# vedantsawal/Cost-and-Carbon-Aware-Kubernetes-Autoscaler

Hardware: AMD Instinct MI355X
Metric: policy-evaluated cluster-steps/sec (higher is better)
Workload: dtype int32+int64+f64; 1 GPU; config2: 1e5 clusters x 1 deployment x 1440 one-minute steps, HPA + peak/off-peak, 16-type catalog; scenarios_per_gpu=100000, steps_per_rollout=1440, mode=trajectory, schedule=lane-skewed (single deployment), trace_layout=wave-tiled [wave][T][lanes] (built by the first rollout), parallelism=scenario-sharded x1

## Files before the change

### cost-and-carbon-aware-kubernetes-autoscaler_amd/csrc/abi_debug.cpp

```cpp
#include <algorithm>
#include <cstdio>
#include <vector>

#include "ctx.h"
#include "host_rules.h"

using namespace ccka;

int stamps_buffer(ccka_ctx* c, unsigned long long** out) {
  if (!c->d_stamps.reserve(12)) return fail(c, CCKA_ENOMEM, "stamps alloc");
  HIPCHK(c, hipMemsetAsync(c->d_stamps, 0, 12 * sizeof(unsigned long long), c->stream));
  *out = c->d_stamps;
  return CCKA_OK;
}

extern "C" {

int ccka_debug_copy_gbs(ccka_ctx* c, int64_t bytes, int32_t reps, double* gbs) {
  if (!c || !gbs || bytes < (1 << 20) || reps < 1 || reps > 64) return CCKA_EINVAL;
  (void)hipSetDevice(c->device);
  bytes &= ~(int64_t)4095;
  DevBuf<char> a, b;
  if (!a.resize(bytes) || !b.resize(bytes))
    return fail(c, CCKA_ENOMEM, "copy probe alloc (2 x %lld bytes)", (long long)bytes);
// ... 28 lines not shown

int ccka_debug_engine(ccka_ctx* c, int32_t mode) {
  if (!c || mode < 0 || mode > 3) return CCKA_EINVAL;
  c->sk_coop_f2 = mode == 3;
  c->engine_mode = mode == 3 ? 0 : mode;
  return CCKA_OK;
}

int ccka_debug_last_engine(ccka_ctx* c, int32_t* engine, double* table_ms) {
  if (!c) return CCKA_EINVAL;
  if (engine) *engine = c->last_engine;
  if (table_ms) *table_ms = c->last_table_ms;
  return CCKA_OK;
}

int ccka_debug_last_plan(ccka_ctx* c, int32_t out[12]) {
  static_assert(PLAN_FIELDS == 12, "ccka_debug_last_plan's out[12]");
  if (!c || !out) return CCKA_EINVAL;
  if (!c->ran || c->last_engine == 3 || c->last_engine == 4) return fail(c, CCKA_ESTATE, "no whole-horizon rollout ran last");
  std::copy(c->last_plan, c->last_plan + PLAN_FIELDS, out);
  return CCKA_OK;
}

int ccka_debug_pg_chunk(ccka_ctx* c, int64_t rows) {
  if (!c || rows < 0) return CCKA_EINVAL;
  c->pg_chunk = rows;
  return CCKA_OK;
}

int ccka_debug_policy_table(ccka_ctx* c, int32_t on) {
  if (!c) return CCKA_EINVAL;
  c->pol_table_off = on == 0;
  return CCKA_OK;
}

int ccka_debug_policy_fused(ccka_ctx* c, int32_t on) {
  if (!c) return CCKA_EINVAL;
  c->pol_fused_off = on == 0;
  return CCKA_OK;
}

int ccka_debug_policy_graph(ccka_ctx* c, int32_t on) {
  if (!c) return CCKA_EINVAL;
  c->pol_graph_off = on == 0;
  return CCKA_OK;
}

int ccka_debug_lpw(ccka_ctx* c, int32_t lpw) {
  if (!c || lpw < 0 || lpw > 64) return CCKA_EINVAL;
  c->lpw = lpw;
  return CCKA_OK;
}

int ccka_debug_trace_flat(ccka_ctx* c, int32_t on) {
  if (!c) return CCKA_EINVAL;
  c->trace_flat = on != 0;
  return CCKA_OK;
}

int ccka_debug_occ(ccka_ctx* c, int32_t occ) {
  if (!c || occ < 0 || occ > 3 || occ == 1) return CCKA_EINVAL;
  c->occ = occ;
  return CCKA_OK;
}

int ccka_debug_mlp_tile(ccka_ctx* c, int32_t tile) {
  if (!c || (tile != 16 && tile != 32)) return CCKA_EINVAL;
  c->mlp_tile = tile;
  return CCKA_OK;
}

int ccka_debug_mlp_stamps(ccka_ctx* c, int32_t enable) {
  if (!c) return CCKA_EINVAL;
  c->mlp_stamps = enable != 0;
  return CCKA_OK;
}

int ccka_debug_stamps(ccka_ctx* c, unsigned long long* out8) {
  if (!c || !out8 || !c->d_stamps) return CCKA_EINVAL;
  HIPCHK(c, hipMemcpy(out8, c->d_stamps, 12 * sizeof(unsigned long long), hipMemcpyDeviceToHost));
  return CCKA_OK;
}

int ccka_debug_totals(ccka_ctx* c, const int64_t* cost, const int32_t* slo, const int64_t* pend_min,
                      const int32_t* nmin_spot, const int32_t* nmin_od, const int32_t* launches,
                      const int32_t* deletions, const double* energy, const double* gco2, int64_t n,
                      ccka_totals* out) {
  if (!c || !cost || !slo || !pend_min || !nmin_spot || !nmin_od || !launches || !deletions || !energy || !gco2 ||
      !out || n < 1 || n > (int64_t)1 << 31)
    return CCKA_EINVAL;
  (void)hipSetDevice(c->device);
  DevBuf<char> d_res;
  if (!d_res.resize(carve_results(nullptr, n, nullptr))) return fail(c, CCKA_ENOMEM, "totals columns (%lld)", (long long)n);
  ResultPtrs r{};
  carve_results(d_res, n, &r);
  struct { void* dst; const void* src; size_t sz; } m[] = {
      {r.cost, cost, 8}, {r.slo, slo, 4}, {r.pend_min, pend_min, 8}, {r.nmin_spot, nmin_spot, 4},
      {r.nmin_od, nmin_od, 4}, {r.launches, launches, 4}, {r.deletions, deletions, 4}, {r.energy, energy, 8},
      {r.gco2, gco2, 8}};
  for (auto& x : m) HIPCHK(c, hipMemcpyAsync(x.dst, x.src, (size_t)n * x.sz, hipMemcpyHostToDevice, c->stream));
  const int rc = totals_of(c, r, n, out);
  (void)hipStreamSynchronize(c->stream);
  return rc;
}

int ccka_debug_traj_stage(ccka_ctx* c, int64_t records) {
// ... 33 lines not shown
```

### cost-and-carbon-aware-kubernetes-autoscaler_amd/csrc/abi_rollout.cpp

```cpp
#include <algorithm>
#include <cstddef>
#include <cstring>

#include "ctx.h"
#include "host_rules.h"

using namespace ccka;

static int32_t d1_lpw(const ccka_ctx* c) {
  if (c->lpw > 0) return c->lpw;
  const int64_t slots = 2LL * 4 * c->cus;
  return (int32_t)std::min<int64_t>(64, std::max<int64_t>(32, (c->N + slots - 1) / slots));
}

static int d1_trace_tile(ccka_ctx* c) {
  if (!c->d1_world || c->hw.n_deploy != 1 || c->n_traces > 0 || !c->have_load) return CCKA_OK;
  const int32_t lpw = d1_lpw(c);
  if (c->load_w_lpw == lpw && c->d_load_w) return CCKA_OK;
  const int64_t cnt = trace_tile_count(c->N, c->hw.n_steps, lpw);
  c->load_w_lpw = 0;
  if (!c->d_load_w.resize(cnt)) return CCKA_OK;
  HIPCHK(c, launch_trace_tile(c->d_load, c->d_load_w, c->N, c->hw.n_steps, lpw, c->stream));
  HIPCHK(c, hipStreamSynchronize(c->stream));
  c->load_w_lpw = lpw;
// ... 132 lines not shown
  if (dmax > 4) return false;
  if (k.nsub != 1 || k.hlen != 0 || !k.all_hours || (k.ablate & ~16) != 0) return false;
  if (w.disrupt_ext & (CCKA_DISRUPT_DRIFT | CCKA_DISRUPT_REPLACE | CCKA_DISRUPT_MULTI)) return false;
  for (int d = 0; d < w.n_deploy; ++d) {
    const int sc = w.deploy[d].scaler;
    if (sc != CCKA_SCALER_HPA && sc != CCKA_SCALER_STATIC) return false;
    if (sc != CCKA_SCALER_HPA) continue;
    const ccka_deployment& dp = w.deploy[d];
    if (dp.target_util_pct <= 0 || dp.target_util_pct > kSkMax16) return false;
    if (!(dp.tolerance >= 0.0 && dp.tolerance < 1.0)) return false;
    if (dp.max_replicas > kSkMax16 || dp.replicas0 > kSkMax16) return false;
  }
  if (c->sc_target_max > kSkMax16 || c->sc_maxr_max > kSkMax16) return false;
  return true;
}

extern "C" {

int ccka_rollout_async(ccka_ctx* c, int32_t trajectory) {
  if (!c) return CCKA_EINVAL;
  if (!c->have_world || !c->have_sc) return fail(c, CCKA_ESTATE, "world/scenarios not set");
  if (!c->have_load) return fail(c, CCKA_ESTATE, "no load traces (ccka_set_load / ccka_gen_load)");
  (void)hipSetDevice(c->device);
  const ccka_world& w = c->hw;
  int block = 256;
  size_t lds = 0;
  int rc;
  KParams k;
  if ((rc = setup_general(c, trajectory, k, &block, &lds)) != CCKA_OK) return rc;
  int32_t* const plan = c->last_plan;
  std::fill(plan, plan + PLAN_FIELDS, -1);
  plan[PLAN_TRACE_MOD] = k.trace_mod != 0;
  if (c->engine_mode == 0 && c->d1_world && !c->d1_ready && (rc = d1_prepare(c)) != CCKA_OK) return rc;
  if (c->engine_mode == 0 && c->d1_world && c->d1_ok && !c->detail_on) {
    const TableParams tp = table_params(c, c->d_wc1000, c->NW, c->d_table, c->d_jtab);
    D1Params p = c->d1;
    p.load = c->d_load; p.price = c->d_price; p.ci_gpwmin = c->d_ci_gpwmin; p.acc = c->d_acc;
    p.table = c->d_table; p.jtab = c->d_jtab;
    p.region = c->d_region; p.target = c->d_target; p.maxr = c->d_maxr; p.down_stab = c->d_dstab;
    p.reset_ca = c->d_resetca; p.pswitch = c->d_pswitch; p.wci = c->d_wci; p.cap_sel = c->d_capsel;
    p.res = k.res; p.traj = k.traj;
    p.N = c->N;
    p.NL = k.NL;
    p.trace_mod = k.trace_mod;
    p.first_id = k.first_id;
    p.NW = c->NW;
    p.occ = c->occ > 0 ? c->occ : 2;
    p.lpw = d1_lpw(c);
    if (!c->trace_flat) {
      if ((rc = d1_trace_tile(c)) != CCKA_OK) return rc;
      if (c->load_w_lpw == p.lpw && c->d_load_w && p.trace_mod == 0) p.load_w = c->d_load_w;
    }
    p.ablate = k.ablate;
    if ((k.ablate & 16) && (rc = stamps_buffer(c, &p.stamps)) != CCKA_OK) return rc;
    HIPCHK(c, hipEventRecord(c->ev0, c->stream));
    HIPCHK(c, launch_table(tp, c->stream));
    if (p.replace || p.multi) {
      TableParams t2 = tp;
      t2.wc1000 = c->d_wc0;
      t2.NW = 1;
      t2.offer = 1;
      t2.table = c->d_table2;
      t2.jtab = c->d_jtab2;
      HIPCHK(c, launch_table(t2, c->stream));
      p.table2 = c->d_table2;
    }
    HIPCHK(c, hipEventRecord(c->ev_mid, c->stream));
    HIPCHK(c, launch_rollout_d1(p, c->stream, plan));
    plan[PLAN_D1_NW] = c->NW;
    plan[PLAN_D1_NZI] = p.NZI;
    plan[PLAN_D1_JT] = p.JT;
    HIPCHK(c, hipEventRecord(c->ev1, c->stream));
    c->last_engine = 2;
    c->traj_nt = true;
  } else {
    if ((k.ablate & 16) && (rc = stamps_buffer(c, &k.stamps)) != CCKA_OK) return rc;
    const bool sk = sk_eligible(c, k);
    if (sk) {
      if ((rc = sk_trace(c)) != CCKA_OK) return rc;
      if (c->load_nt_dp) k.load_nt = c->d_load_nt;
      int dmax, nmax;
      kernel_dims(w.n_deploy, w.max_nodes, &dmax, &nmax);
      const size_t col = ((lds + 15) & ~(size_t)15), need = (size_t)nmax * (7 + dmax) * block * 4;
      if (!c->sk_coop_f2 && rollout_sk_lane_f2() && w.n_types <= 64 && col + need <= 160 * 1024) {
        k.lds_lclaims = (int32_t)col;
        lds = col + need;
      }
    }
    HIPCHK(c, hipEventRecord(c->ev0, c->stream));
    HIPCHK(c, hipEventRecord(c->ev_mid, c->stream));
    if (sk) HIPCHK(c, launch_rollout_sk(k, block, lds, c->stream));
    else HIPCHK(c, launch_rollout(k, block, lds, c->stream));
    HIPCHK(c, hipEventRecord(c->ev1, c->stream));
    plan[PLAN_GRID] = (int32_t)((c->N + block - 1) / block);
    plan[PLAN_SPAN] = k.span;
    plan[PLAN_ALL_HOURS] = k.all_hours;
    plan[PLAN_HLEN] = k.hlen;
    plan[PLAN_LDS] = (int32_t)lds;
    plan[PLAN_LCLAIMS] = k.lds_lclaims >= 0;
    c->last_engine = sk ? 5 : 1;
    c->traj_nt = sk;
  }
  c->traj_valid = trajectory != 0;
  c->detail_valid = c->detail_on;
  c->ran = true;
  return CCKA_OK;
}

int ccka_set_detail(ccka_ctx* c, int32_t on) {
  if (!c) return CCKA_EINVAL;
  c->detail_on = on != 0;
  return CCKA_OK;
}

int ccka_get_detail(ccka_ctx* c, ccka_detail* out, int64_t count) {
  if (!c || !out) return CCKA_EINVAL;
  if (!c->ran || !c->detail_valid) return fail(c, CCKA_ESTATE, "last rollout recorded no detail (ccka_set_detail)");
  if (count != c->N) return fail(c, CCKA_EINVAL, "detail count %lld != %lld scenarios", (long long)count, (long long)c->N);
  (void)hipSetDevice(c->device);
  HIPCHK(c, hipMemcpy2DAsync(out, sizeof(ccka_detail), c->d_detail, sizeof(DetailDev), sizeof(ccka_detail), (size_t)count,
                             hipMemcpyDeviceToHost, c->stream));
  HIPCHK(c, hipStreamSynchronize(c->stream));
  return CCKA_OK;
}
// ... 199 lines not shown
```

### cost-and-carbon-aware-kubernetes-autoscaler_amd/csrc/ctx.h

```cpp
#pragma once
#include <hip/hip_runtime.h>
#include <rccl/rccl.h>

#include <cstdint>
#include <string>
#include <vector>

#include "../../include/ccka.h"
#include "devbuf.h"
#include "kparams.h"

#pragma GCC visibility push(hidden)

struct ccka_ctx {
  template <class T>
  using Buf = ccka::DevBuf<T>;

  int device = 0;
  hipStream_t stream = nullptr;
  hipEvent_t ev0 = nullptr, ev_mid = nullptr, ev1 = nullptr;
  std::string err;
  int cus = 0;
  char name[128] = {0};
  bool have_world = false;
// ... 17 lines not shown
  Buf<uint8_t> d_capsel;
  Buf<int32_t> d_load;
  bool have_load = false;
  Buf<int32_t> d_load_w;
  int32_t load_w_lpw = 0;
  Buf<int32_t> d_load_nt;
  int32_t load_nt_dp = 0;
  bool trace_flat = false;
  Buf<char> d_res;
  ccka::ResultPtrs res{};
  Buf<ccka_traj_rec> d_traj;
  bool traj_valid = false;
  bool traj_nt = false;
  Buf<ccka_traj_rec> d_traj_t;
  int64_t traj_stage = 0;
  Buf<long long> d_parts;
  Buf<ccka_totals> d_totals;
  Buf<int32_t> d_sinq;
  ncclComm_t comm = nullptr;
  double last_ms = 0.0;
  double last_table_ms = 0.0;
  bool ran = false;
  bool d1_world = false;
  bool d1_ready = false;
  bool d1_ok = false;
  bool sc_maxr_ok = true;
  int sc_dstab_max = -1;
  int sc_target_max = -1;
  int sc_maxr_max = -1;
  Buf<int2> d_hist;
  uint32_t sc_capsel_or = 0;
  int sc_pswitch_any = -1;
  ccka::D1Params d1{};
  std::vector<uint32_t> zmasks;
  std::vector<double> h_cw;
  Buf<long long> d_acc;
  Buf<int32_t> d_order;
  Buf<int32_t> d_cap1s;
  Buf<int32_t> d_cap1t;
  Buf<uint32_t> d_zmasks;
  Buf<double> d_wc1000;
  Buf<uint8_t> d_wci;
  Buf<int2> d_table;
  Buf<int32_t> d_jtab;
  Buf<int2> d_table2;
  Buf<int32_t> d_jtab2;
  Buf<double> d_wc0;
  int JT = 0, NW = 0;
  int engine_mode = 0;
  bool sk_coop_f2 = false;
  int32_t ablate = 0;
  Buf<unsigned long long> d_stamps;
  int lpw = 0;
  int occ = 0;
  int mlp_stamps = 0;
  Buf<ccka_grid_stats> d_gstats;
  Buf<ccka_grid_stats> d_gcand;
  Buf<ccka_grid_stats> d_ggather;
  Buf<int64_t> d_gcounts;
  Buf<int32_t> d_gn;
  Buf<uint8_t> d_gflags;
  Buf<ccka_grid_stats> d_gfront;
  Buf<ccka_timeline_row> d_tlrows;
  Buf<int64_t> d_snap;
  bool have_snap = false;
  int64_t snap_first = 0, snap_n = 0, snap_grid_size = 0, snap_traces = 0;
  Buf<ccka_paired_row> d_prows;
  Buf<uint32_t> d_pflag;
  bool mlp_have_w = false;
  Buf<ccka::mlp_bf16x8> d_w1f;
  Buf<ccka::mlp_bf16x8> d_w2f;
  Buf<ccka::mlp_bf16x8> d_w3f;
  Buf<ccka::mlp_bf16x8> d_w1g;
  Buf<ccka::mlp_bf16x8> d_w2g;
  Buf<ccka::mlp_bf16x8> d_w3g;
  int mlp_tile = 16;
  Buf<float> d_mb;
  Buf<uint16_t> d_mx;
  Buf<float> d_my;
  int64_t mlp_n = 0;
  int last_engine = 0;
  int32_t last_plan[ccka::PLAN_FIELDS] = {0};
  Buf<int32_t> d_pol_state;
  Buf<int16_t> d_pol_target;
  Buf<double> d_pol_cw;
  Buf<int16_t> d_rec_target;
  Buf<double> d_rec_cw;
  bool pol_rec_valid = false;
  bool pol_feat_on = false;
  hipGraphExec_t pol_graph = nullptr;
  std::vector<unsigned char> pol_graph_key;
  bool pol_graph_off = false;
  bool pol_fused_off = false;
  bool pol_table_off = false;
  int64_t pg_chunk = 0;
  int64_t pg_mpad = 0;
  Buf<int2> d_ptable;
  Buf<int32_t> d_pjtab;
  Buf<double> d_pwc;
  Buf<uint16_t> d_feat_rec;
  Buf<ccka::mlp_bf16x8> d_w2b;
  Buf<ccka::mlp_bf16x8> d_w3b;
  Buf<uint8_t> d_pg_act;
  Buf<float> d_pg_coef;
  Buf<uint64_t> d_pg_seed;
  uint64_t pg_seed_host = 0;
// ... 45 lines not shown
```

### cost-and-carbon-aware-kubernetes-autoscaler_amd/csrc/host_rules.h

```cpp
#pragma once
#include <cstdint>

#include "../../include/ccka.h"

namespace ccka {

inline const char* trace_gen_invalid(const ccka_trace_gen& g) {
  typedef __int128 i128;
  const int64_t wb = (int64_t)g.base_hi - g.base_lo, wa = (int64_t)g.amp_hi_pm - g.amp_lo_pm;
  if (wb < 0 || wa < 0) return "a range has hi < lo";
  if (wb + 1 > INT32_MAX || wa + 1 > INT32_MAX) return "a range's width + 1 exceeds int32";
  if (g.burst_len < 0) return "burst_len < 0";
  if (g.burst_len > INT32_MAX - 1439) return "bstart + burst_len can exceed int32";
  auto mag = [](int32_t lo, int32_t hi) {
    const i128 a = lo < 0 ? -(i128)lo : (i128)lo, b = hi < 0 ? -(i128)hi : (i128)hi;
    return a > b ? a : b;
  };
  const i128 lim = INT64_MAX;
  const i128 B = mag(g.base_lo, g.base_hi), A = mag(g.amp_lo_pm, g.amp_hi_pm);
  const i128 P1 = B * (65536000 + 65536 * A);
  if (P1 > lim) return "base * (65536000 + amp * SIN) can leave int64";
  const i128 V1 = P1 / 65536000;
  const i128 P2 = V1 * (37837000 + 131072 * mag(g.noise_pm, g.noise_pm));
  if (P2 > lim) return "v * (37837000 + noise * e) can leave int64";
  const i128 V2 = P2 / 37837000;
  if (V2 * mag(g.burst_mult_pm, g.burst_mult_pm) > lim) return "v * burst_mult can leave int64";
  return nullptr;
}

constexpr int32_t kMaxStartMinute = INT32_MAX - 65535;
constexpr int32_t kMaxProvisionDelay = 0x7ffffffe - 65534;

inline const char* world_timing_invalid(const ccka_world& w) {
  if (w.n_steps < 1 || w.n_steps > 65535) return "n_steps out of range";
  if (w.start_minute < 0 || w.provision_delay_steps < 0) return "negative timing";
  if (w.start_minute > kMaxStartMinute) return "start_minute + n_steps can leave int32";
  if (w.provision_delay_steps > kMaxProvisionDelay) return "a ready step t + provision_delay_steps can reach 0x7fffffff";
  if (w.peak_start_min < 0 || w.peak_start_min > 1440) return "peak_start_min outside [0, 1440]";
  if (w.peak_end_min < 0 || w.peak_end_min > 1440) return "peak_end_min outside [0, 1440]";
  return nullptr;
}

constexpr int64_t kTrajStageRecs = int64_t(4) << 20;

inline int64_t traj_stage_cap(int64_t N, int64_t count, int64_t stage) {
  const int64_t lim = stage > 0 ? stage : kTrajStageRecs;
  const int64_t cap = count < lim ? count : lim;
  return cap > N ? cap : N;
}

inline int64_t trace_tile_count(int64_t N, int64_t T, int64_t lpw) { return T * ((N + lpw - 1) / lpw * lpw); }
inline int64_t trace_nt_count(int64_t NL, int64_t T, int64_t DP) { return NL * T * DP; }

}
```

### cost-and-carbon-aware-kubernetes-autoscaler_amd/csrc/kparams.h

```cpp
#pragma once
#include <hip/hip_runtime.h>
#include <stddef.h>
#include <stdint.h>

#include "../../include/ccka.h"

namespace ccka {

struct DetailDev {
  ccka_detail d;
  int64_t e_hour[CCKA_MAX_POOLS];
  int64_t base_e_hour;
};

__host__ __device__ constexpr int64_t state_words(int dmax, int nmax) {
  return (int64_t)dmax * (5 + 2 * CCKA_HIST) + 5 * CCKA_MAX_POOLS + (int64_t)nmax * (6 + dmax) + 36;
}

__host__ __device__ constexpr int hist_entries(int window_s, int sync_s) {
  return window_s > sync_s ? (window_s - 1) / sync_s : 0;
}

struct ResultPtrs {
  int64_t* cost;
// ... 139 lines not shown
struct D1Patch {
  int32_t policy, cas, zi, cm;
};

struct D1Params {
  const int32_t* load;
  const int32_t* load_w;
  const int32_t* price;
  const double* ci_gpwmin;
  const long long* acc;
  const int2* table;
  const int32_t* jtab;
  const uint8_t* region;
  const int16_t* target;
  const int16_t* maxr;
  const int16_t* down_stab;
  const int16_t* reset_ca;
  const uint8_t* pswitch;
  const uint8_t* wci;
  const uint8_t* cap_sel;
  ResultPtrs res;
  ccka_traj_rec* traj;
  int64_t N;
  int64_t NL, trace_mod, first_id;
  int32_t lpw;
  int32_t occ;
  int32_t bdef;
  int32_t T, K, Z, R, NP, maxn, NZI, NW, JT;
  int32_t start_minute, peak_start, peak_end, pswitch0, delay;
  int32_t base_nodes, base_type, slo_util, pdb_pct, pdb_member;
  int32_t replicas0, minr, maxr0, target0, req_cpu, limit, dstab0, reset_ca0, capsel0;
  double tol_lo, tol_hi;
  long long base_nw;
  int32_t ablate;
  unsigned long long* stamps;
  D1Rule up, dn;
  int32_t budget[CCKA_MAX_POOLS];
  D1Patch patch[CCKA_MAX_POOLS][4];
  int32_t drift;
  uint32_t zml[16];
  int32_t drift_on;
  int32_t replace;
  const int2* table2;
  int32_t lds_tab;
  int32_t nsub;
  int32_t he4;
  int32_t multi;
  int32_t keda;
  int32_t k_thr;
  int32_t k_act;
  int32_t k_cds;
  int32_t k_min;
  int32_t k_max;
};
static_assert(sizeof(D1Params) == 1048 && offsetof(D1Params, traj) == 232, "D1Params: the kernels' argument layout");

struct TableParams {
  const int32_t* price;
  const double* ci_gpwh;
  const ccka_itype* types;
  const int32_t* order;
  const int32_t* cap1s;
  const int32_t* cap1t;
  const uint32_t* zmasks;
  const double* wc1000;
  int2* table;
  int32_t* jtab;
  int32_t K, Z, R, NZI, NW, JT;
  int32_t offer;
};

hipError_t launch_table(const TableParams& t, hipStream_t s);
hipError_t launch_trace_tile(const int32_t* in, int32_t* out, int64_t N, int64_t T, int32_t lpw, hipStream_t s);

struct GridSrc {
  const int64_t* cost;
  const double* gco2;
  const int32_t* slo;
  const double* energy;
  int64_t grid_size, first_grid, n_grids;
};
hipError_t launch_grid_stats(const GridSrc& g, ccka_grid_stats* out, hipStream_t s);
struct GridSel {
  GridSrc g;
  int64_t rank[4];
  int32_t kind[4];
};
hipError_t launch_grid_select(const GridSel& q, ccka_grid_stats* out, hipStream_t s);
hipError_t launch_copy16(const void* in, void* out, int64_t bytes, int cus, hipStream_t s);
hipError_t launch_pareto(const ccka_grid_stats* in, int n, const int32_t* n_dev, uint8_t* flags,
                         ccka_grid_stats* out, int32_t* count_dev, hipStream_t s);
hipError_t launch_pareto_union(const ccka_grid_stats* gathered, const int64_t* counts, int ranks, int cap,
                               ccka_grid_stats* out, int32_t* n_dev, hipStream_t s);

struct MlpParams {
  const uint16_t* x;
  float* y;
  const mlp_bf16x8* w1f;
  const mlp_bf16x8* w2f;
  const mlp_bf16x8* w3f;
  const float *b1, *b2, *b3;
  int64_t N;
  unsigned long long* stamps;
  const mlp_bf16x8* w1g;
  const mlp_bf16x8* w2g;
  const mlp_bf16x8* w3g;
};
hipError_t launch_mlp(const MlpParams& p, int cus, hipStream_t s);
// ... 91 lines not shown
```

### cost-and-carbon-aware-kubernetes-autoscaler_amd/csrc/rollout_d1.hip

```cpp
#include <hip/hip_runtime.h>
#include <stdint.h>

#include "../../include/ccka.h"
#include "d1_common.h"
#include "kparams.h"

#pragma clang fp contract(off)

namespace ccka {

namespace {

struct Best {
  double s;
  int k;
  int info;
  int price;
};

__device__ __forceinline__ bool better(double s2, int k2, double s, int k) {
  return s2 < s || (s2 == s && k2 < k);
}

__device__ __forceinline__ void take_if_better(Best& a, const Best& b) {
  if (better(b.s, b.k, a.s, a.k)) a = b;
}

__device__ __forceinline__ Best shfl_up_best(const Best& a, int off) {
  Best o;
  o.s = __shfl_up(a.s, off);
  o.k = __shfl_up(a.k, off);
  o.info = __shfl_up(a.info, off);
  o.price = __shfl_up(a.price, off);
  return o;
}

__device__ __forceinline__ Best readlane_best(const Best& a, int l) {
  Best o;
  const long long b = __double_as_longlong(a.s);
  const int lo = __builtin_amdgcn_readlane((int)(b & 0xffffffffLL), l);
  const int hi = __builtin_amdgcn_readlane((int)(b >> 32), l);
  o.s = __longlong_as_double(((long long)hi << 32) | (unsigned int)lo);
  o.k = __builtin_amdgcn_readlane(a.k, l);
  o.info = __builtin_amdgcn_readlane(a.info, l);
  o.price = __builtin_amdgcn_readlane(a.price, l);
  return o;
}

}

__global__ void __launch_bounds__(256) table_kernel(TableParams q) {
  const int lane = threadIdx.x & (WAVE - 1);
  const int64_t key = ((int64_t)blockIdx.x * blockDim.x + threadIdx.x) / WAVE;
  const int64_t nkeys = (int64_t)q.R * 24 * q.NZI * 3 * q.NW;
  if (key >= nkeys) return;
  int64_t x = key;
  const int wi = (int)(x % q.NW); x /= q.NW;
// ... 71 lines not shown
  for (int q = 0; q < 2; ++q) {
    o.type[q] = opq(r.type[q]);
    o.value[q] = opq(r.value[q]);
    o.pmask[q] = opq(r.pmask[q]);
    o.factor[q] = opq(r.factor[q]);
  }
#pragma unroll
  for (int w = 0; w < 4; ++w) {
    o.stab16[w] = opq(r.stab16[w]);
    o.pm16[0][w] = opq(r.pm16[0][w]);
    o.pm16[1][w] = opq(r.pm16[1][w]);
  }
  return o;
}

__device__ __forceinline__ int rate_limit1(const D1Rule& R, bool up, int cur, const uint32_t* del) {
  if (R.sel == CCKA_SELECT_DISABLED) return cur;
  const bool min_sel = R.sel == CCKA_SELECT_MIN;
  long long res = (up == min_sel) ? 0x7fffffffLL : -0x80000000LL;
#pragma unroll
  for (int q = 0; q < 2; ++q) {
    if (q >= R.n) break;
    int added = 0, removed = 0;
    if (R.pmask[q]) {
      const short2v z = {0, 0};
#pragma unroll
      for (int w = 0; w < 4; ++w) {
        const short2v d = as_s2(del[w]), m = as_s2((uint32_t)R.pm16[q][w]);
        added = __builtin_amdgcn_sdot2(__builtin_elementwise_max(d, z), m, added, false);
        removed = __builtin_amdgcn_sdot2(__builtin_elementwise_max(z - d, z), m, removed, false);
      }
    }
    const long long pst = (long long)cur - added + removed;
    long long pr;
    if (R.type[q] == CCKA_HPA_PODS) pr = up ? pst + R.value[q] : pst - R.value[q];
    else if (up) pr = (int)ceil((double)pst * R.factor[q]);
    else pr = (int)((double)pst * R.factor[q]);
    res = (up == min_sel) ? min(res, pr) : max(res, pr);
  }
  return (int)res;
}

}

#define D1_STAMP(k)                                          \
  if constexpr (STAMPS) {                                    \
    __builtin_amdgcn_sched_barrier(0);                       \
    const uint64_t now_ = __builtin_amdgcn_s_memtime();      \
    __builtin_amdgcn_sched_barrier(0);                       \
    st_acc[k] += now_ - st_last;                             \
    st_last = now_;                                          \
  }

constexpr int D1_RB = 64;
constexpr int D1_K = 2;
constexpr int D1_VMN = 4;
constexpr int D1_S = 8;
constexpr int D1_BACK = CCKA_HIST;
static_assert(D1_VMN + 4 * D1_S + D1_BACK <= D1_RB && D1_RB - D1_S - D1_BACK - D1_VMN >= 2 * D1_S,
              "ring too small for the DMA lead");
constexpr int D1_RING_BYTES = D1_RB * WAVE * 4;
constexpr int D1_PRIO_HI = 3;
__device__ __forceinline__ void d1_dma_row(const int32_t* src, uint32_t lds_row) {
  unsigned keep;
  asm volatile(
      "s_mov_b32 %0, m0\n\t"
      "s_mov_b32 m0, %2\n\t"
      "s_nop 0\n\t"
      "global_load_lds_dword %1, off\n\t"
      "s_mov_b32 m0, %0"
      : "=&s"(keep)
      : "v"(src), "s"(lds_row)
      : "memory");
}
__device__ __forceinline__ void d1_wait_rows() { asm volatile("s_waitcnt vmcnt(%0)" ::"n"(D1_VMN) : "memory"); }
__device__ __forceinline__ void d1_wait_all() { asm volatile("s_waitcnt vmcnt(0)" ::: "memory"); }

__device__ __forceinline__ uint32_t xcd_block(uint32_t b, uint32_t n) {
  const uint32_t x = b & 7u, k = b >> 3, q = n >> 3, r = n & 7u;
  return x * q + min(x, r) + k;
}

template <int MAXN, int MAXP, bool STAMPS, int OCC, bool BDEF, bool DRIFT = false, int NSUB = 1, int HE = 8,
          bool G3 = false, bool KEDA = false>
__global__ void __launch_bounds__(256, OCC) rollout_d1_kernel(D1Params p) {
  static_assert(NSUB == 1 || (NSUB == 4 && BDEF), "15 s sync: lean default path");
  static_assert(!KEDA || (BDEF && NSUB == 1 && !DRIFT), "KEDA: default behavior, one decision per step");
  static_assert(HE == 8 || (HE == 4 && NSUB == 1 && BDEF), "4-record ring: default behavior, one decision per step");
  static_assert(!G3 || (DRIFT && MAXP == 2), "G3: the DRIFT instantiation, two pools");
  constexpr int HW = NSUB == 1 ? HE / 2 : 10;
  constexpr int JR = NSUB == 1 ? HE : 5;
  uint64_t st_acc[12] = {0, 0, 0, 0, 0, 0, 0, 0, 0, 0, 0, 0};
  uint64_t st_last = STAMPS ? __builtin_amdgcn_s_memtime() : 0;
  extern __shared__ __attribute__((aligned(16))) int4 s_acc[];
  for (int x = threadIdx.x; x < p.K; x += blockDim.x) {
    const long long idle = p.acc[x * 3 + 0];
    s_acc[x] = make_int4((int)(idle & 0xffffffffLL), (int)(idle >> 32), (int)p.acc[x * 3 + 1], (int)p.acc[x * 3 + 2]);
  }
  const bool ldt = p.lds_tab;
  const uint32_t tab_off = ((uint32_t)p.K * 16u + 255u) / 256u * 256u + (blockDim.x / WAVE) * (uint32_t)D1_RING_BYTES;
  const int n_pr = p.R * 24 * p.K * p.Z * 2;
  const int n_pr8 = (n_pr + 1) & ~1;
  int* const s_price = reinterpret_cast<int*>(reinterpret_cast<char*>(s_acc) + tab_off);
  double* const s_ci = reinterpret_cast<double*>(s_price + n_pr8);
  int* const s_jtab = reinterpret_cast<int*>(s_ci + p.R * 24);
  if (ldt) {
    for (int x = threadIdx.x; x < n_pr; x += blockDim.x) s_price[x] = p.price[x];
    for (int x = threadIdx.x; x < p.R * 24; x += blockDim.x) s_ci[x] = p.ci_gpwmin[x];
    for (int x = threadIdx.x; x < p.R * 24 * p.NZI * 3; x += blockDim.x) s_jtab[x] = p.jtab[x];
  }
  __syncthreads();
  const int lane = threadIdx.x & (WAVE - 1);
  const int64_t wv = (int64_t)xcd_block(blockIdx.x, gridDim.x) * (blockDim.x / WAVE) + (threadIdx.x / WAVE);
  const int64_t i = wv * p.lpw + lane;
  if (lane >= p.lpw || i >= p.N) return;

  const int r = p.region ? (int)p.region[i] : 0;
  const int target = KEDA ? 1 : (p.target ? (int)p.target[i] : p.target0);
  const int mx = KEDA ? opq(p.k_max) : (p.maxr ? (int)p.maxr[i] : p.maxr0);
  const int dwin = (!KEDA && p.down_stab) ? (int)p.down_stab[i] : p.dstab0;
  const int nd = min(NSUB == 1 ? __popc(window_mask(dwin)) : (dwin > 15 ? (dwin - 1) / 15 : 0), 2 * HW);
  const int dnmask = NSUB == 1 ? window_mask(dwin) : 0;
  const int reset_ca = p.reset_ca ? (int)p.reset_ca[i] : p.reset_ca0;
  const int pswitch = p.pswitch ? (int)p.pswitch[i] : p.pswitch0;
  const int wi = p.wci ? (int)p.wci[i] : 0;
  const uint32_t capsel = p.cap_sel ? (uint32_t)p.cap_sel[i] : (uint32_t)p.capsel0;
  const int minr = KEDA ? max(opq(p.k_min), 1) : opq(p.minr), req = opq(p.req_cpu), limit = opq(p.limit);
  const int kthr = KEDA ? opq(p.k_thr) : 1, kact = KEDA ? opq(p.k_act) : 0, kcds = KEDA ? opq(p.k_cds) : 0;
  const bool kmin0 = KEDA && opq(p.k_min) == 0;
  const float rkthr = __builtin_amdgcn_rcpf((float)kthr);
  int ulo = max(0, (int)floor(p.tol_lo * (double)target) - 2);
  while ((double)ulo / (double)target < p.tol_lo) ++ulo;
  int uhi = (int)floor(p.tol_hi * (double)target) + 2;
  while ((double)uhi / (double)target > p.tol_hi) --uhi;
  const float rtarget = __builtin_amdgcn_rcpf((float)target);

  const int NP = opq(p.NP), NZI = opq(p.NZI), NW = opq(p.NW), JT = opq(p.JT);
  const int maxn = opq(p.maxn), ablate = CCKA_ABLATE_BUILD ? opq(p.ablate) : 0, pdb_member = opq(p.pdb_member);
  const int pdb_pct = opq(p.pdb_pct), slo_util = opq(p.slo_util), delay = opq(p.delay);
  const int base_nodes = opq(p.base_nodes), base_type = opq(p.base_type);
  const int K = opq(p.K), Z = opq(p.Z), T = opq(p.T);
  const int ps = opq(p.peak_start) % 1440, pe = opq(p.peak_end) % 1440;
  const int ps_raw = opq(p.peak_start), pe_raw = opq(p.peak_end);
  const int sm0 = opq(p.start_minute) % 1440;
  const long long base_nw = opq(p.base_nw);
  const GLOBAL_AS int32_t* const price = opq_ptr(p.price);
  const GLOBAL_AS double* const ci_gpwmin = opq_ptr(p.ci_gpwmin);
  const GLOBAL_AS int2* const table = opq_ptr(p.table);
  const GLOBAL_AS int2* const table2 = opq_ptr(p.table2);
  const int drift_on = opq(p.drift_on), replace = opq(p.replace), multi = G3 ? opq(p.multi) : 0;
  const GLOBAL_AS int32_t* const jtab = opq_ptr(p.jtab);
  GLOBAL_AS int4* const traj = opq_ptr(reinterpret_cast<int4*>(p.traj));
  const D1Rule rup = [&] { if constexpr (BDEF) return d1_default_rule(true); else return opq_rule(p.up); }();
// ... 255 lines not shown
    if (__builtin_expect(slow, 0)) upp = usage / max(rpods, 1);
    return rpods > 0 ? upp : 0;
  };
  auto dyn_energy = [&](int upp) -> long long {
    if (__builtin_expect(upp <= 0xFFFF, 1)) {
      unsigned long long ed = 0;
#pragma unroll
      for (int n = 0; n < MAXN; ++n) {
        const uint32_t use = min((uint32_t)spods[n] * (uint32_t)upp, alloc_ready(n));
        ed += (unsigned long long)dyn_of(n) * use;
      }
      return (long long)ed;
    }
    long long e = 0;
#pragma unroll
    for (int n = 0; n < MAXN; ++n) {
      const uint64_t prod = (uint64_t)(uint32_t)spods[n] * (uint64_t)(uint32_t)upp;
      const uint32_t al = alloc_ready(n);
      const uint32_t use = prod < (uint64_t)al ? (uint32_t)prod : al;
      e += (long long)((uint64_t)dyn_of(n) * use);
    }
    return e;
  };

  int t = 0;
  int nxt = 0;
  int npb = 0;
  int tq = 0;
  bool stall = false;
  auto flush = [&](int upto) {
    const int n = upto - tq;
    cost += (burn + base_price) * (long long)n;
    e_hour += (base_nw + Isum) * (long long)n;
    if constexpr (BDEF) {
      e_hour += (long long)(Ssum * (unsigned long long)usum);
      usum = 0;
    }
    pend_min += (replicas - rpods) * n;
    nmin_spot += nsp * n;
    nmin_od += nod * n;
    tq = upto;
  };

  const int64_t wtb = [&] {
    const int64_t x = wv * p.lpw;
    const uint32_t hi = (uint32_t)__builtin_amdgcn_readfirstlane((int)(x >> 32));
    const uint32_t lo = (uint32_t)__builtin_amdgcn_readfirstlane((int)(x & 0xffffffffLL));
    return (int64_t)(((uint64_t)hi << 32) | lo);
  }();
  const int32_t* lp = p.load_w ? p.load_w + wtb * T + lane
                               : p.load + (p.trace_mod > 0 ? (p.first_id + i) % p.trace_mod : i);
  const long long lsl = opq(p.load_w ? (long long)p.lpw : (long long)p.NL);
  const uint32_t ring_off = (uint32_t)__builtin_amdgcn_readfirstlane(
      (int)(((uint32_t)p.K * 16u + 255u) / 256u * 256u + (threadIdx.x / WAVE) * (uint32_t)D1_RING_BYTES));
  const uint32_t ring_lds = (uint32_t)(uintptr_t)s_acc + ring_off;
  const int* const ring = reinterpret_cast<const int*>(reinterpret_cast<const char*>(s_acc) + ring_off);
  constexpr int rsw = WAVE, rbn = D1_RB;
  auto rrow = [&](int x) { return x & (D1_RB - 1); };
  auto ridx = [&](int r) { return r * rsw + lane; };
  auto rnext = [&](int r, int q) { return (r + q) & (D1_RB - 1); };
  int tf = 0;
  int tfr = 0;
  const int32_t* lpf = lp;
  auto tf_adv = [&]() {
    ++tf;
    ++tfr;
    if (tfr == rbn) tfr = 0;
    lpf += lsl;
  };
  {
    const int n0 = min(T, D1_VMN + 4 * D1_S);
    while (tf < n0) {
      d1_dma_row(lpf, (uint32_t)__builtin_amdgcn_readfirstlane((int)(ring_lds + (uint32_t)tfr * (uint32_t)(rsw * 4))));
      tf_adv();
    }
    d1_wait_all();
  }
  int t_rdy = tf;
  bool pf_ok = false;
  bool qadv = true;
  int Lpf[D1_S];
#pragma unroll
  for (int q = 0; q < D1_S; ++q) Lpf[q] = 0;
  const int64_t w0 = wtb;
  const int wlanes = (int)min((int64_t)p.lpw, p.N - w0);
  const __amdgpu_buffer_rsrc_t trs = __builtin_amdgcn_make_buffer_rsrc(
      traj ? (void*)(reinterpret_cast<int4*>(p.traj) + w0 * T) : (void*)p.load, 0, traj ? wlanes * T * 16 : 0,
      0x00020000);
  const int lb = lane * T * 16;

  for (int it = 0;; ++it) {
    const bool live = t < T;
    if (__ballot(live) == 0) break;
    d1_wait_rows();
    t_rdy = max(t_rdy, tf - D1_VMN);
    const uint64_t sb = __ballot(stall);
    if constexpr (STAMPS) st_acc[9] += 1;
    if (sb != 0 && (it % D1_K == D1_K - 1 || !qadv)) {
      __builtin_amdgcn_s_setprio(0);
      if constexpr (STAMPS) { st_acc[10] += 1; st_acc[11] += __popcll(sb); }
      const bool ev = stall;
      int L = 0, minute = 0, rh = 0, pd = 0, step_last_type = 0xFFFF;
      int4 rec;
      uint32_t flags = 0;
      bool g_acted = false, hchg = false, jchg = false;
      uint32_t emp_e = 0, weou_e = 0;
      HpaOut hp{};
      if (ev) {
        stall = false;
        const int tr = rrow(t);
        L = ring[ridx(tr)];
        if constexpr (BDEF) {
          const int kq = min(t - tq, wr);
          if (kq > 0) {
            const int cur16 = min(replicas, D1_REC_SAT);
            int us[JR], rv[JR];
            bool anylow = false;
#pragma unroll
            for (int j = 0; j < JR; ++j) {
              us[j] = KEDA ? ring[ridx(rnext(tr, rbn - 1 - j))] : min(ring[ridx(rnext(tr, rbn - 1 - j))], q_rcap);
              rv[j] = q_met ? cur16 : (int)0x8000;
              anylow |= (j < kq) & q_met & (us[j] < q_pge);
            }
            if (KEDA && anylow) {
#pragma unroll
              for (int j = 0; j < JR; ++j) {
// ... 863 lines not shown
          q_slo = slo_thr;
          q_rbp = rpods > 0 ? __builtin_amdgcn_rcpf((float)rpods) : 0.f;
          q_hbp = 0.5f * q_rbp;
          q_usat = Rmax > 0.f ? (int)fminf(0.9999f * __builtin_amdgcn_rcpf(Rmax), 1073741824.0f) - 1 : 0x7fffffff;
          q_pendv = replicas - rpods;
          q_nodes = (nsp & 0xFFFF) | nod << 16;
          q_w0 = 0xFFFF | (int)((q_peak ? 1u : 0u) << 16);
          q_w1 = q_w0 | (8 << 16);
        } else {
          q_rbd = __builtin_amdgcn_rcpf((float)(rpods * req));
          q_rbc = __builtin_amdgcn_rcpf((float)(replicas * req));
        }
        if constexpr (BDEF) {
          int hit = -0x40000000;
#pragma unroll
          for (int k = 2 * HW - 1; k >= 0; --k) {
            const int e = (int)(short)(hdn[k >> 1] >> (16 * (k & 1)));
            hit = e >= replicas ? t - k / NSUB : hit;
          }
          q_hold = replicas <= minr ? 0x3fffffff : hit + wl;
          if (!q_met) q_hold = 0x3fffffff;
        }
        {
          const int th = t + 60 - minute % 60;
          int nx = min(next_ready, th);
          if (pswitch) {
            if (t >= npb) {
              const int dps = (ps - minute + 1439) % 1440 + 1, dpe = (pe - minute + 1439) % 1440 + 1;
              npb = t + min(dps, dpe);
            }
            nx = min(nx, npb);
          }
          const uint32_t gm = rdy & (emp_e | (Ffree >= minscap ? weou_e : (weou_e & ~cmask)) |
                                     ((DRIFT && replace) ? (weou_e & od_slots() & ~emp_e & ~srcm) : 0u) |
                                     ((DRIFT && G3 && multi) ? (weou_e & ~emp_e & ~taint()) : 0u));
#pragma unroll
          for (int n = 0; n < MAXN; ++n) nx = ((gm >> n & 1u) && slc[n] > t) ? min(nx, slc[n]) : nx;
          if (g_acted || ablated(ablate, 15)) nx = t + 1;
          nxt = nx;
        }
      }
      if (ev) {
        d1_store_rec(trs, lb + t * 16, rec);
        ++t;
      }
      pf_ok = pf_ok && !ev;
      D1_STAMP(7);
    }
    __builtin_amdgcn_s_setprio(D1_PRIO_HI);
    if (tf < T) {
      if (__ballot(t < T && t < tf + D1_S - rbn + D1_BACK) == 0) {
        const int n1 = min(T, tf + D1_S);
        while (tf < n1) {
          d1_dma_row(lpf, (uint32_t)__builtin_amdgcn_readfirstlane((int)(ring_lds + (uint32_t)tfr * (uint32_t)(rsw * 4))));
          tf_adv();
        }
        if (tf == T) {
          d1_wait_all();
          t_rdy = T;
        }
      }
    }
    bool adv = false;
    if (!pf_ok) {
      const int tr = rrow(t);
#pragma unroll
      for (int q = 0; q < D1_S; ++q) Lpf[q] = ring[ridx(rnext(tr, q))];
    }

    D1_STAMP(8);
    const int tlim = min(T, t_rdy);
#pragma unroll
    for (int sub = 0; sub < D1_S; ++sub) {
    if constexpr (BDEF) {
        const int L = Lpf[sub];
        const int usage = min(L, q_rcap);
        const int cv = KEDA ? L : usage;
        const bool ge = cv >= q_pge;
        bool ok = (t < nxt) & ((uint32_t)cv < (uint32_t)q_ulim) & (ge | (t <= q_hold));
        const bool kac = KEDA && L > kact;
        if constexpr (KEDA) ok = ok & (!q_kcd | kac | (t < kcd));
        const bool can = !stall & (t < tlim);
        const bool go = ok & can;
        stall = stall | (can & !ok);
        q_hold = (go & ge) ? max(q_hold, t + wl) : q_hold;
        if constexpr (KEDA) kcd = (go & kac) ? t + kcds : kcd;
        const int upp = (int)fmaf((float)usage, q_rbp, q_hbp);
        if (__builtin_expect(go & (upp > q_usat), 0)) {
          const long long corr = dyn_energy(upp) - (long long)(Ssum * (unsigned long long)(uint32_t)upp);
          e_hour += corr;
        }
        usum += go ? (uint32_t)upp : 0u;
        const bool slo_b = usage >= q_slo;
        slo += (go & slo_b) ? 1 : 0;
        d1_store_rec(trs, go ? lb + t * 16 : D1_NOSTORE, make_int4(replicas, q_pendv, q_nodes, slo_b ? q_w1 : q_w0));
        t += go ? 1 : 0;
        adv = adv | go;
    } else
    if (t < T && !stall && t < t_rdy) {
      const int L = Lpf[sub];
      int4 rec;
      if (!(stall = t >= nxt)) {
        const HpaOut h = hpa_eval(L, replicas, rpods, q_rbd, q_rbc);
        stall = h.desired != replicas;
        if (!stall) {
          hpa_commit(h, replicas);
          const int upp = upp_of(L, q_rbp);
// ... 8 lines not shown
          d1_store_rec(trs, lb + t * 16, rec);
          ++t;
        }
      }
    }
    }
    qadv = __ballot(adv) != 0;
    D1_STAMP(1);
    pf_ok = t + (D1_S - 1) < t_rdy;
    {
      const int tr = rrow(t);
#pragma unroll
      for (int q = 0; q < D1_S; ++q) Lpf[q] = ring[ridx(rnext(tr, q))];
    }
    D1_STAMP(8);
  }
  d1_wait_all();
  if constexpr (STAMPS) {
    if (lane == (__ffsll((long long)__ballot(1)) - 1)) {
      for (int k = 1; k < 12; ++k) atomicAdd(&p.stamps[k], (unsigned long long)st_acc[k]);
      atomicMax(&p.stamps[0], (unsigned long long)st_acc[9]);
    }
  }
  flush(T);
  energy_nw += e_hour;
  gco2 += (double)e_hour * (ci_min * 1e-9);
  p.res.cost[i] = cost;
  p.res.energy[i] = (double)energy_nw * 1e-9;
  p.res.gco2[i] = gco2;
  p.res.slo[i] = slo;
  p.res.pend_min[i] = pend_min;
  p.res.nmin_spot[i] = nmin_spot;
  p.res.nmin_od[i] = nmin_od;
  p.res.launches[i] = launches;
  p.res.deletions[i] = deletions;
  p.res.peak_nodes[i] = peak_nodes;
  p.res.final_reps[i] = replicas;
  p.res.final_nodes[i] = __popc(used);
  p.res.last_choice[i] = last_choice;
  p.res.hash[i] = hash;
}

hipError_t launch_table(const TableParams& t, hipStream_t s) {
  const int64_t nkeys = (int64_t)t.R * 24 * t.NZI * 3 * t.NW;
  const unsigned grid = (unsigned)((nkeys * WAVE + 255) / 256);
  hipLaunchKernelGGL(table_kernel, dim3(grid), dim3(256), 0, s, t);
  return hipGetLastError();
}

hipError_t launch_rollout_d1(const D1Params& p, hipStream_t s, int32_t* plan) {
  const int B = 256;
  const int64_t waves = (p.N + p.lpw - 1) / p.lpw;
  const unsigned grid = (unsigned)((waves + B / WAVE - 1) / (B / WAVE));
  size_t lds = ((size_t)p.K * sizeof(int4) + 255) / 256 * 256 + (size_t)(B / WAVE) * D1_RING_BYTES;
  const size_t npr = (size_t)p.R * 24 * p.K * p.Z * 2;
  const size_t tabB = ((npr + 1) & ~(size_t)1) * 4 + (size_t)p.R * 24 * 8 + (size_t)p.R * 24 * p.NZI * 3 * 4;
  D1Params q = p;
  q.lds_tab = 0;
  if (lds + tabB <= 80 * 1024) {
    q.lds_tab = 1;
    lds += tabB;
  }
  auto go = [&](auto kernel) { hipLaunchKernelGGL(kernel, dim3(grid), dim3(B), lds, s, q); };
  const bool d = p.bdef != 0;
  int inst = 802;
  if (p.keda) {
    if (p.he4) go(rollout_d1_kernel<8, 2, false, 2, true, false, 1, 4, false, true>);
    else go(rollout_d1_kernel<8, 2, false, 2, true, false, 1, 8, false, true>);
  } else if (p.nsub == 4) {
    if (p.multi) go(rollout_d1_kernel<8, 2, false, 2, true, true, 4, 8, true>);
    else if (p.drift) go(rollout_d1_kernel<8, 2, false, 2, true, true, 4>);
    else go(rollout_d1_kernel<8, 2, false, 2, true, false, 4>);
  } else if (p.multi) {
    if (d) go(rollout_d1_kernel<8, 2, false, 2, true, true, 1, 8, true>);
    else go(rollout_d1_kernel<8, 2, false, 2, false, true, 1, 8, true>);
  } else if (p.drift) {
    if (d) go(rollout_d1_kernel<8, 2, false, 2, true, true>);
    else go(rollout_d1_kernel<8, 2, false, 2, false, true>);
  } else if (p.stamps) {
    if (d && p.he4) go(rollout_d1_kernel<8, 2, true, 2, true, false, 1, 4>);
    else if (d) go(rollout_d1_kernel<8, 2, true, 2, true>);
    else go(rollout_d1_kernel<8, 2, true, 2, false>);
  } else if (p.maxn <= 8 && p.NP <= 2 && p.occ == 3) {
    go(rollout_d1_kernel<8, 2, false, 3, false>);
  } else if (p.maxn <= 8 && p.NP <= 2) {
    if (d && p.he4) go(rollout_d1_kernel<8, 2, false, 2, true, false, 1, 4>);
    else if (d) go(rollout_d1_kernel<8, 2, false, 2, true>);
    else go(rollout_d1_kernel<8, 2, false, 2, false>);
  } else if (p.maxn <= 8) {
    inst = 804;
    go(rollout_d1_kernel<8, 4, false, 2, false>);
  } else if (p.NP <= 2) {
    inst = 1602;
    go(rollout_d1_kernel<16, 2, false, 1, false>);
  } else {
    inst = 1604;
    go(rollout_d1_kernel<16, 4, false, 1, false>);
  }
  if (plan) {
    plan[PLAN_GRID] = (int32_t)grid;
    plan[PLAN_LDS] = (int32_t)lds;
    plan[PLAN_D1_LDS_TAB] = q.lds_tab;
    plan[PLAN_D1_INST] = inst;
  }
  return hipGetLastError();
}

}
```

Baseline: 76.90 billion cluster-steps/s.

## Size the d1 trace ring from spare LDS with a lane-count pitch

```diff
diff --git a/cost-and-carbon-aware-kubernetes-autoscaler_amd/csrc/abi_debug.cpp b/cost-and-carbon-aware-kubernetes-autoscaler_amd/csrc/abi_debug.cpp
--- a/cost-and-carbon-aware-kubernetes-autoscaler_amd/csrc/abi_debug.cpp
+++ b/cost-and-carbon-aware-kubernetes-autoscaler_amd/csrc/abi_debug.cpp
@@ -104,6 +104,27 @@
   return CCKA_OK;
 }
 
+int ccka_debug_d1_ring_rows(ccka_ctx* c, int32_t rows) {
+  if (!c || rows < 0) return CCKA_EINVAL;
+  c->d1_ring_rows = rows;
+  return CCKA_OK;
+}
+
+int ccka_debug_d1_ring(ccka_ctx* c, int32_t* rows, int32_t* pitch) {
+  if (!c) return CCKA_EINVAL;
+  if (!c->ran || c->last_engine != 2) return fail(c, CCKA_ESTATE, "no single-deployment rollout ran last");
+  if (rows) *rows = c->d1_ring_last[0];
+  if (pitch) *pitch = c->d1_ring_last[1];
+  return CCKA_OK;
+}
+
+int ccka_debug_d1_geometry(int32_t K, int32_t R, int32_t Z, int32_t NZI, int32_t lpw, int32_t out[5]) {
+  if (!out || K < 1 || K > 1024 || R < 1 || Z < 1 || NZI < 1 || lpw < 1 || lpw > 64) return CCKA_EINVAL;
+  const D1Geometry g = d1_geometry(K, R, Z, NZI, lpw, 0);
+  out[0] = g.lds_tab; out[1] = g.rows; out[2] = g.pitch; out[3] = g.ring_bytes; out[4] = g.lds;
+  return CCKA_OK;
+}
+
 int ccka_debug_trace_flat(ccka_ctx* c, int32_t on) {
   if (!c) return CCKA_EINVAL;
   c->trace_flat = on != 0;
diff --git a/cost-and-carbon-aware-kubernetes-autoscaler_amd/csrc/abi_rollout.cpp b/cost-and-carbon-aware-kubernetes-autoscaler_amd/csrc/abi_rollout.cpp
--- a/cost-and-carbon-aware-kubernetes-autoscaler_amd/csrc/abi_rollout.cpp
+++ b/cost-and-carbon-aware-kubernetes-autoscaler_amd/csrc/abi_rollout.cpp
@@ -208,6 +208,11 @@
       if (c->load_w_lpw == p.lpw && c->d_load_w && p.trace_mod == 0) p.load_w = c->d_load_w;
     }
     p.ablate = k.ablate;
+    p.ring_rows = c->d1_ring_rows;
+    if (p.ring_rows != 0 && !d1_ring_rows_ok(p.K, p.R, p.Z, p.NZI, p.lpw, p.ring_rows))
+      return fail(c, CCKA_EINVAL, "forced ring rows %d outside [%d, %d]", p.ring_rows, kD1RingRowsMin,
+                  d1_geometry(p.K, p.R, p.Z, p.NZI, p.lpw, 0).rows);
+    const D1Geometry geo = d1_geometry(p.K, p.R, p.Z, p.NZI, p.lpw, p.ring_rows);
     if ((k.ablate & 16) && (rc = stamps_buffer(c, &p.stamps)) != CCKA_OK) return rc;
     HIPCHK(c, hipEventRecord(c->ev0, c->stream));
     HIPCHK(c, launch_table(tp, c->stream));
@@ -226,6 +231,8 @@
     plan[PLAN_D1_NW] = c->NW;
     plan[PLAN_D1_NZI] = p.NZI;
     plan[PLAN_D1_JT] = p.JT;
+    c->d1_ring_last[0] = geo.rows;
+    c->d1_ring_last[1] = geo.pitch;
     HIPCHK(c, hipEventRecord(c->ev1, c->stream));
     c->last_engine = 2;
     c->traj_nt = true;
diff --git a/cost-and-carbon-aware-kubernetes-autoscaler_amd/csrc/ctx.h b/cost-and-carbon-aware-kubernetes-autoscaler_amd/csrc/ctx.h
--- a/cost-and-carbon-aware-kubernetes-autoscaler_amd/csrc/ctx.h
+++ b/cost-and-carbon-aware-kubernetes-autoscaler_amd/csrc/ctx.h
@@ -93,6 +93,8 @@
   int32_t ablate = 0;
   Buf<unsigned long long> d_stamps;
   int lpw = 0;
+  int d1_ring_rows = 0;
+  int32_t d1_ring_last[2] = {0, 0};
   int occ = 0;
   int mlp_stamps = 0;
   Buf<ccka_grid_stats> d_gstats;
diff --git a/cost-and-carbon-aware-kubernetes-autoscaler_amd/csrc/host_rules.h b/cost-and-carbon-aware-kubernetes-autoscaler_amd/csrc/host_rules.h
--- a/cost-and-carbon-aware-kubernetes-autoscaler_amd/csrc/host_rules.h
+++ b/cost-and-carbon-aware-kubernetes-autoscaler_amd/csrc/host_rules.h
@@ -52,4 +52,39 @@
 inline int64_t trace_tile_count(int64_t N, int64_t T, int64_t lpw) { return T * ((N + lpw - 1) / lpw * lpw); }
 inline int64_t trace_nt_count(int64_t NL, int64_t T, int64_t DP) { return NL * T * DP; }
 
+constexpr int32_t kD1Waves = 4;
+constexpr int32_t kD1LdsBudget = 80 * 1024;
+constexpr int32_t kD1RingRowsMin = 48;
+constexpr int32_t kD1RingRowsMax = 512;
+struct D1Geometry {
+  int32_t lds_tab;
+  int32_t rows;
+  int32_t pitch;
+  int32_t ring_bytes;
+  int32_t lds;
+};
+inline int32_t d1_catalog_bytes(int32_t K) { return (K * 16 + 255) / 256 * 256; }
+inline int64_t d1_table_bytes(int32_t K, int32_t R, int32_t Z, int32_t NZI) {
+  const int64_t npr = (int64_t)R * 24 * K * Z * 2;
+  return ((npr + 1) & ~(int64_t)1) * 4 + (int64_t)R * 24 * 8 + (int64_t)R * 24 * NZI * 3 * 4;
 }
+inline int32_t d1_ring_bytes(int32_t rows, int32_t pitch) { return ((rows - 1) * pitch + 256 + 15) & ~15; }
+inline D1Geometry d1_geometry(int32_t K, int32_t R, int32_t Z, int32_t NZI, int32_t lpw, int32_t rows) {
+  D1Geometry g{};
+  const int32_t cat = d1_catalog_bytes(K);
+  const int64_t tabB = d1_table_bytes(K, R, Z, NZI);
+  g.lds_tab = cat + kD1Waves * 64 * 256 + tabB <= kD1LdsBudget;
+  const int32_t tab = g.lds_tab ? (int32_t)tabB : 0;
+  g.pitch = lpw * 4;
+  const int32_t per_wave = ((kD1LdsBudget - cat - tab) / kD1Waves) & ~15;
+  const int32_t fit = per_wave >= 256 ? (per_wave - 256) / g.pitch + 1 : 0;
+  g.rows = rows > 0 ? rows : (fit < 64 ? 64 : (fit > kD1RingRowsMax ? kD1RingRowsMax : fit));
+  g.ring_bytes = d1_ring_bytes(g.rows, g.pitch);
+  g.lds = cat + kD1Waves * g.ring_bytes + tab;
+  return g;
+}
+inline bool d1_ring_rows_ok(int32_t K, int32_t R, int32_t Z, int32_t NZI, int32_t lpw, int32_t rows) {
+  return rows >= kD1RingRowsMin && rows <= d1_geometry(K, R, Z, NZI, lpw, 0).rows;
+}
+
+}
diff --git a/cost-and-carbon-aware-kubernetes-autoscaler_amd/csrc/kparams.h b/cost-and-carbon-aware-kubernetes-autoscaler_amd/csrc/kparams.h
--- a/cost-and-carbon-aware-kubernetes-autoscaler_amd/csrc/kparams.h
+++ b/cost-and-carbon-aware-kubernetes-autoscaler_amd/csrc/kparams.h
@@ -215,8 +215,11 @@
   int32_t k_cds;
   int32_t k_min;
   int32_t k_max;
-};
-static_assert(sizeof(D1Params) == 1048 && offsetof(D1Params, traj) == 232, "D1Params: the kernels' argument layout");
+  int32_t ring_rows;
+  int32_t ring_pitch;
+  int32_t ring_bytes;
+};
+static_assert(sizeof(D1Params) == 1064 && offsetof(D1Params, traj) == 232, "D1Params: the kernels' argument layout");
 
 struct TableParams {
   const int32_t* price;
diff --git a/cost-and-carbon-aware-kubernetes-autoscaler_amd/csrc/rollout_d1.hip b/cost-and-carbon-aware-kubernetes-autoscaler_amd/csrc/rollout_d1.hip
--- a/cost-and-carbon-aware-kubernetes-autoscaler_amd/csrc/rollout_d1.hip
+++ b/cost-and-carbon-aware-kubernetes-autoscaler_amd/csrc/rollout_d1.hip
@@ -3,6 +3,7 @@
 
 #include "../../include/ccka.h"
 #include "d1_common.h"
+#include "host_rules.h"
 #include "kparams.h"
 
 #pragma clang fp contract(off)
@@ -180,14 +181,14 @@
     st_last = now_;                                          \
   }
 
-constexpr int D1_RB = 64;
 constexpr int D1_K = 2;
 constexpr int D1_VMN = 4;
 constexpr int D1_S = 8;
 constexpr int D1_BACK = CCKA_HIST;
-static_assert(D1_VMN + 4 * D1_S + D1_BACK <= D1_RB && D1_RB - D1_S - D1_BACK - D1_VMN >= 2 * D1_S,
+constexpr int D1_ROWS_MIN = 48;
+static_assert(D1_VMN + 4 * D1_S + D1_BACK <= D1_ROWS_MIN && D1_ROWS_MIN - D1_S - D1_BACK - D1_VMN >= 2 * D1_S &&
+                  D1_ROWS_MIN == kD1RingRowsMin,
               "ring too small for the DMA lead");
-constexpr int D1_RING_BYTES = D1_RB * WAVE * 4;
 constexpr int D1_PRIO_HI = 3;
 __device__ __forceinline__ void d1_dma_row(const int32_t* src, uint32_t lds_row) {
   unsigned keep;
@@ -226,7 +227,7 @@
     s_acc[x] = make_int4((int)(idle & 0xffffffffLL), (int)(idle >> 32), (int)p.acc[x * 3 + 1], (int)p.acc[x * 3 + 2]);
   }
   const bool ldt = p.lds_tab;
-  const uint32_t tab_off = ((uint32_t)p.K * 16u + 255u) / 256u * 256u + (blockDim.x / WAVE) * (uint32_t)D1_RING_BYTES;
+  const uint32_t tab_off = ((uint32_t)p.K * 16u + 255u) / 256u * 256u + (blockDim.x / WAVE) * (uint32_t)p.ring_bytes;
   const int n_pr = p.R * 24 * p.K * p.Z * 2;
   const int n_pr8 = (n_pr + 1) & ~1;
   int* const s_price = reinterpret_cast<int*>(reinterpret_cast<char*>(s_acc) + tab_off);
@@ -588,15 +589,21 @@
                                : p.load + (p.trace_mod > 0 ? (p.first_id + i) % p.trace_mod : i);
   const long long lsl = opq(p.load_w ? (long long)p.lpw : (long long)p.NL);
   const uint32_t ring_off = (uint32_t)__builtin_amdgcn_readfirstlane(
-      (int)(((uint32_t)p.K * 16u + 255u) / 256u * 256u + (threadIdx.x / WAVE) * (uint32_t)D1_RING_BYTES));
+      (int)(((uint32_t)p.K * 16u + 255u) / 256u * 256u + (threadIdx.x / WAVE) * (uint32_t)p.ring_bytes));
   const uint32_t ring_lds = (uint32_t)(uintptr_t)s_acc + ring_off;
   const int* const ring = reinterpret_cast<const int*>(reinterpret_cast<const char*>(s_acc) + ring_off);
-  constexpr int rsw = WAVE, rbn = D1_RB;
-  auto rrow = [&](int x) { return x & (D1_RB - 1); };
-  auto ridx = [&](int r) { return r * rsw + lane; };
-  auto rnext = [&](int r, int q) { return (r + q) & (D1_RB - 1); };
+  const int rsw = p.ring_pitch >> 2, rbn = p.ring_rows;
   int tf = 0;
   int tfr = 0;
+  auto rrow = [&](int x) {
+    const uint32_t r = (uint32_t)(tfr - (tf - x));
+    return (int)min(r, r + (uint32_t)rbn);
+  };
+  auto ridx = [&](int r) { return __mul24(r, rsw) + lane; };
+  auto rnext = [&](int r, int q) {
+    const uint32_t a = (uint32_t)(r + q);
+    return (int)min(a, a - (uint32_t)rbn);
+  };
   const int32_t* lpf = lp;
   auto tf_adv = [&]() {
     ++tf;
@@ -607,7 +614,7 @@
   {
     const int n0 = min(T, D1_VMN + 4 * D1_S);
     while (tf < n0) {
-      d1_dma_row(lpf, (uint32_t)__builtin_amdgcn_readfirstlane((int)(ring_lds + (uint32_t)tfr * (uint32_t)(rsw * 4))));
+      d1_dma_row(lpf, (uint32_t)__builtin_amdgcn_readfirstlane((int)(ring_lds + (uint32_t)tfr * (uint32_t)p.ring_pitch)));
       tf_adv();
     }
     d1_wait_all();
@@ -1577,7 +1584,7 @@
       if (__ballot(t < T && t < tf + D1_S - rbn + D1_BACK) == 0) {
         const int n1 = min(T, tf + D1_S);
         while (tf < n1) {
-          d1_dma_row(lpf, (uint32_t)__builtin_amdgcn_readfirstlane((int)(ring_lds + (uint32_t)tfr * (uint32_t)(rsw * 4))));
+          d1_dma_row(lpf, (uint32_t)__builtin_amdgcn_readfirstlane((int)(ring_lds + (uint32_t)tfr * (uint32_t)p.ring_pitch)));
           tf_adv();
         }
         if (tf == T) {
@@ -1692,15 +1699,16 @@
   const int B = 256;
   const int64_t waves = (p.N + p.lpw - 1) / p.lpw;
   const unsigned grid = (unsigned)((waves + B / WAVE - 1) / (B / WAVE));
-  size_t lds = ((size_t)p.K * sizeof(int4) + 255) / 256 * 256 + (size_t)(B / WAVE) * D1_RING_BYTES;
-  const size_t npr = (size_t)p.R * 24 * p.K * p.Z * 2;
-  const size_t tabB = ((npr + 1) & ~(size_t)1) * 4 + (size_t)p.R * 24 * 8 + (size_t)p.R * 24 * p.NZI * 3 * 4;
+  static_assert(B / WAVE == kD1Waves, "d1_geometry's waves per block");
+  if (p.lpw < 1 || p.lpw > WAVE || (p.ring_rows != 0 && !d1_ring_rows_ok(p.K, p.R, p.Z, p.NZI, p.lpw, p.ring_rows)))
+    return hipErrorInvalidValue;
+  const D1Geometry g = d1_geometry(p.K, p.R, p.Z, p.NZI, p.lpw, p.ring_rows);
+  const size_t lds = (size_t)g.lds;
   D1Params q = p;
-  q.lds_tab = 0;
-  if (lds + tabB <= 80 * 1024) {
-    q.lds_tab = 1;
-    lds += tabB;
-  }
+  q.lds_tab = g.lds_tab;
+  q.ring_rows = g.rows;
+  q.ring_pitch = g.pitch;
+  q.ring_bytes = g.ring_bytes;
   auto go = [&](auto kernel) { hipLaunchKernelGGL(kernel, dim3(grid), dim3(B), lds, s, q); };
   const bool d = p.bdef != 0;
   int inst = 802;
```

After: 77.07 billion cluster-steps/s (median of 2 runs). Within noise of the previous version (+0.2%).
